# kubeflow/mpi-operator

Hardware: AMD Instinct MI355X
Metric: images/sec (higher is better)
Workload: dtype bf16; 1 GPU; model=resnet101, global_batch=64, image=224, parallelism=dp1, impl=hip, graph=True

## Files before the change

mpi_operator_amd/ops/_backend.py:

```python
from __future__ import annotations

import importlib
import os
import sys

_ext = None
_ext_err: Exception | None = None


def _try_load():
    global _ext, _ext_err
    if _ext is not None or _ext_err is not None:
        return
    try:
        import torch

        _ext = importlib.import_module("mpi_operator_amd.ops._mpi_amd_hip")
        if os.environ.get("MPIAMD_EPI_VEC", "1") == "0":
            _ext.set_epilogue_vec(False)
    except Exception as e:
        _ext_err = e


def hip_ext():
    _try_load()
    if _ext is None:
        raise RuntimeError(
            "mpi_operator_amd HIP extension (_mpi_amd_hip.so) is not available "
            "but a GPU op was requested. Build it in-tree with "
            "`python -m mpi_operator_amd.ops.build_hip` (hipcc, gfx950). "
            f"Original import error: {_ext_err!r}"
        )
    return _ext


def hip_available() -> bool:
    _try_load()
    return _ext is not None
```

mpi_operator_amd/ops/csrc/batchnorm.hip:

```cpp
#include "common.h"
#include "knobs.h"
#include "launchers.h"

template <int WHAT>
__global__ void bn_partials_k(const ushort8 *__restrict__ x,
                              const ushort8 *__restrict__ dy,
                              const ushort8 *__restrict__ y,
                              const uint8_t *__restrict__ mask,
                              const float *__restrict__ mean,
                              const float *__restrict__ invstd,
                              float *__restrict__ partial,
                              long M, int C8, int relu) {
  int C = C8 * 8;
  int cb = threadIdx.x % C8;
  int row_lane = threadIdx.x / C8;
  int rows_per_block = blockDim.x / C8;
  float a0[8] = {0}, a1[8] = {0};
  float mn[8], is[8];
  if (WHAT == 1 && row_lane < rows_per_block) {
#pragma unroll
    for (int j = 0; j < 8; ++j) {
      mn[j] = mean[cb * 8 + j];
      is[j] = invstd[cb * 8 + j];
    }
  }
  if (row_lane < rows_per_block) {
    long stride = (long)gridDim.x * rows_per_block;
    for (long row = (long)blockIdx.x * rows_per_block + row_lane; row < M;
         row += 2 * stride) {
      long r2 = row + stride;
      bool has2 = r2 < M;
      long off = row * C8 + cb, off2 = r2 * C8 + cb;
      float fx[8], fx2[8];
      ushort8 vx = x[off];
      ushort8 vx2 = has2 ? x[off2] : ushort8{0, 0, 0, 0, 0, 0, 0, 0};
      bf8_to_f8(vx, fx);
      bf8_to_f8(vx2, fx2);
      if (WHAT == 0) {
#pragma unroll
        for (int j = 0; j < 8; ++j) {
          a0[j] += fx[j] + fx2[j];
          a1[j] += fx[j] * fx[j] + fx2[j] * fx2[j];
        }
      } else {
        ushort8 vdy = dy[off];
        ushort8 vdy2 = has2 ? dy[off2] : ushort8{0, 0, 0, 0, 0, 0, 0, 0};
        float fdy[8], fdy2[8];
        bf8_to_f8(vdy, fdy);
        bf8_to_f8(vdy2, fdy2);
        if (relu) {
          if (mask) {
            int m1 = mask[off], m2 = has2 ? mask[off2] : 0;
#pragma unroll
            for (int j = 0; j < 8; ++j) {
              if (!(m1 & (1 << j))) fdy[j] = 0.f;
              if (!(m2 & (1 << j))) fdy2[j] = 0.f;
            }
          } else {
            ushort8 vy = y[off];
            ushort8 vy2 = has2 ? y[off2] : ushort8{0, 0, 0, 0, 0, 0, 0, 0};
#pragma unroll
            for (int j = 0; j < 8; ++j) {
              if (!(bf2f(vy[j]) > 0.f)) fdy[j] = 0.f;
              if (!(bf2f(vy2[j]) > 0.f)) fdy2[j] = 0.f;
            }
          }
        }
#pragma unroll
        for (int j = 0; j < 8; ++j) {
          a0[j] += fdy[j] + fdy2[j];
          a1[j] += fdy[j] * ((fx[j] - mn[j]) * is[j]) +
                   fdy2[j] * ((fx2[j] - mn[j]) * is[j]);
        }
      }
    }
  }
  __shared__ float lds[2][256 * 8];
#pragma unroll
  for (int j = 0; j < 8; ++j) {
    lds[0][threadIdx.x * 8 + j] = a0[j];
    lds[1][threadIdx.x * 8 + j] = a1[j];
  }
  __syncthreads();
  if (row_lane == 0) {
    for (int rl = 1; rl < rows_per_block; ++rl) {
// ... 395 lines not shown
      f2[j] = f2[j] * sc[j] + sh[j] + g2[j];
      if (relu) {
        if (f[j] > 0.f) m1 |= 1 << j;
        if (f2[j] > 0.f) m2 |= 1 << j;
        f[j] = fmaxf(f[j], 0.f);
        f2[j] = fmaxf(f2[j], 0.f);
      }
    }
    y[off] = f8_to_bf8(f);
    if (r2 < M) y[off2] = f8_to_bf8(f2);
    if (relu && mask) {
      mask[off] = (uint8_t)m1;
      if (r2 < M) mask[off2] = (uint8_t)m2;
    }
  }
}

__global__ void bn_bwd_apply_k(const ushort8 *__restrict__ dy,
                               const ushort8 *__restrict__ x,
                               const ushort8 *__restrict__ y,
                               const uint8_t *__restrict__ mask,
                               const float *__restrict__ mean,
                               const float *__restrict__ invstd,
                               const float *__restrict__ k1,
                               const float *__restrict__ k2,
                               const float *__restrict__ k3,
                               ushort8 *__restrict__ dx, long M, int C8,
                               int relu) {
  int cb = threadIdx.x % C8;
  int row_lane = threadIdx.x / C8;
  int rows_per_block = blockDim.x / C8;
  if (row_lane >= rows_per_block) return;
  float mn[8], is[8], a[8], b[8], c3[8];
#pragma unroll
  for (int j = 0; j < 8; ++j) {
    int c = cb * 8 + j;
    mn[j] = mean[c];
    is[j] = invstd[c];
    a[j] = k1[c];
    b[j] = k2[c];
    c3[j] = k3[c];
  }
  long stride = (long)gridDim.x * rows_per_block;
  for (long row = (long)blockIdx.x * rows_per_block + row_lane; row < M;
       row += 2 * stride) {
    long r2 = row + stride;
    long off = row * C8 + cb, off2 = r2 * C8 + cb;
    ushort8 vdy = dy[off], vx = x[off];
    ushort8 vdy2 = r2 < M ? dy[off2] : ushort8{0, 0, 0, 0, 0, 0, 0, 0};
    ushort8 vx2 = r2 < M ? x[off2] : ushort8{0, 0, 0, 0, 0, 0, 0, 0};
    float fdy[8], fx[8], fdy2[8], fx2[8];
    bf8_to_f8(vdy, fdy);
    bf8_to_f8(vx, fx);
    bf8_to_f8(vdy2, fdy2);
    bf8_to_f8(vx2, fx2);
    if (relu) {
      if (mask) {
        int m1 = mask[off], m2 = r2 < M ? mask[off2] : 0;
#pragma unroll
        for (int j = 0; j < 8; ++j) {
          if (!(m1 & (1 << j))) fdy[j] = 0.f;
          if (!(m2 & (1 << j))) fdy2[j] = 0.f;
        }
      } else {
        ushort8 vy = y[off];
        ushort8 vy2 = r2 < M ? y[off2] : ushort8{0, 0, 0, 0, 0, 0, 0, 0};
#pragma unroll
        for (int j = 0; j < 8; ++j) {
          if (!(bf2f(vy[j]) > 0.f)) fdy[j] = 0.f;
          if (!(bf2f(vy2[j]) > 0.f)) fdy2[j] = 0.f;
        }
      }
    }
#pragma unroll
    for (int j = 0; j < 8; ++j) {
      fdy[j] = a[j] * fdy[j] - b[j] - c3[j] * ((fx[j] - mn[j]) * is[j]);
      fdy2[j] = a[j] * fdy2[j] - b[j] - c3[j] * ((fx2[j] - mn[j]) * is[j]);
    }
    dx[off] = f8_to_bf8(fdy);
    if (r2 < M) dx[off2] = f8_to_bf8(fdy2);
  }
}

static void bn_geom(long M, int C8, int &grid, int &rows_per_block) {
  rows_per_block = 256 / C8;
  long g = (M + rows_per_block - 1) / rows_per_block;
  long cap = bn_grid_cap();
  grid = (int)(g > cap ? cap : (g < 1 ? 1 : g));
}

static int bn_apply_grid(long M, int C8) {
  const long cap = bn_apply_grid_cap();
  int rpb = 256 / C8;
  long g = (M + rpb - 1) / rpb;
  return (int)(g > cap ? cap : (g < 1 ? 1 : g));
}

extern "C" hipError_t bn_fwd_train_launch(
    const void *x, const void *res, const float *gamma, const float *beta,
    float eps, int relu, void *y, uint8_t *relu_mask, float *mean,
    float *invstd, float *scale, float *shift, float *partial,
    float *running_mean, float *running_var, float momentum, long M, int C,
    hipStream_t s) {
  int C8 = C / 8;
  if (C8 < 1 || C8 > 256) return hipErrorInvalidValue;
  int grid, rpb;
  bn_geom(M, C8, grid, rpb);
  bn_partials_k<0><<<grid, 256, 0, s>>>((const ushort8 *)x, nullptr, nullptr,
                                        nullptr, nullptr, nullptr, partial, M,
                                        C8, 0);
  HIP_KERNEL_CHECK();
  float unbias = M > 1 ? (float)M / (float)(M - 1) : 1.f;
  bn_finalize_fwd_bands_k<<<C, 256, 0, s>>>(
      partial, grid, C, gamma, beta, 1.f / (float)M, eps, mean, invstd, scale,
      shift, running_mean, running_var, momentum, unbias);
  HIP_KERNEL_CHECK();
  bn_apply_k<<<bn_apply_grid(M, C8), 256, 0, s>>>(
      (const ushort8 *)x, (const ushort8 *)res, scale, shift, (ushort8 *)y,
      relu_mask, M, C8, relu);
  HIP_KERNEL_CHECK();
  return hipSuccess;
}

__global__ void bn_finalize_fwd_bands_k(
    const float *__restrict__ partial, int grid, int C,
    const float *__restrict__ gamma, const float *__restrict__ beta,
    float inv_m, float eps, float *__restrict__ mean,
    float *__restrict__ invstd, float *__restrict__ scale,
    float *__restrict__ shift, float *__restrict__ running_mean,
    float *__restrict__ running_var, float momentum, float unbias) {
  int c = blockIdx.x;
  if (c >= C) return;
  float ga = 0.f, be = 0.f, rm = 0.f, rv = 0.f;
  if (threadIdx.x == 0) {
    ga = gamma[c];
    be = beta[c];
    if (running_mean) {
      rm = running_mean[c];
      rv = running_var[c];
    }
  }
  float s = 0.f, sq = 0.f;
  for (int g = threadIdx.x; g < grid; g += 256) {
    s += partial[(long)g * 2 * C + c];
    sq += partial[(long)g * 2 * C + C + c];
  }
  __shared__ float red[2][256 / WAVE];
  s = wave_sum(s);
  sq = wave_sum(sq);
  if ((threadIdx.x & (WAVE - 1)) == 0) {
    red[0][threadIdx.x / WAVE] = s;
    red[1][threadIdx.x / WAVE] = sq;
  }
  __syncthreads();
  if (threadIdx.x != 0) return;
  s = red[0][0] + red[0][1] + red[0][2] + red[0][3];
  sq = red[1][0] + red[1][1] + red[1][2] + red[1][3];
  float mu = s * inv_m;
  float var = fmaxf(sq * inv_m - mu * mu, 0.f);
  float is = rsqrtf(var + eps);
  mean[c] = mu;
  invstd[c] = is;
  float sc = ga * is;
  scale[c] = sc;
  shift[c] = be - mu * sc;
  if (running_mean) {
    running_mean[c] = rm * (1.f - momentum) + mu * momentum;
    running_var[c] = rv * (1.f - momentum) + var * unbias * momentum;
  }
}

extern "C" hipError_t bn_fwd_train_pre_launch(
    const float *pre_partial, int pre_grid, const void *x, const void *res,
    const float *gamma, const float *beta, float eps, int relu, void *y,
    uint8_t *relu_mask, float *mean, float *invstd, float *scale,
    float *shift, float *running_mean, float *running_var, float momentum,
    long M, int C, hipStream_t s) {
  int C8 = C / 8;
  if (C8 < 1 || C8 > 256) return hipErrorInvalidValue;
  float unbias = M > 1 ? (float)M / (float)(M - 1) : 1.f;
  bn_finalize_fwd_bands_k<<<C, 256, 0, s>>>(
      pre_partial, pre_grid, C, gamma, beta, 1.f / (float)M, eps, mean,
      invstd, scale, shift, running_mean, running_var, momentum, unbias);
  HIP_KERNEL_CHECK();
  bn_apply_k<<<bn_apply_grid(M, C8), 256, 0, s>>>(
      (const ushort8 *)x, (const ushort8 *)res, scale, shift, (ushort8 *)y,
      relu_mask, M, C8, relu);
  HIP_KERNEL_CHECK();
  return hipSuccess;
}

extern "C" hipError_t bn_fwd_eval_launch(const void *x, const float *scale,
                                         const float *shift, int relu, void *y,
                                         long M, int C, hipStream_t s) {
  int C8 = C / 8;
  if (C8 < 1 || C8 > 256) return hipErrorInvalidValue;
  int grid, rpb;
  bn_geom(M, C8, grid, rpb);
  bn_apply_k<<<bn_apply_grid(M, C8), 256, 0, s>>>(
      (const ushort8 *)x, nullptr, scale, shift, (ushort8 *)y, nullptr, M, C8,
      relu);
  HIP_KERNEL_CHECK();
  return hipSuccess;
}

extern "C" hipError_t bn_bwd_launch(const void *dy, const void *x,
                                    const void *y, const uint8_t *relu_mask,
                                    const float *gamma, const float *mean,
                                    const float *invstd, int relu, void *dx,
                                    float *dgamma, float *dbeta, float *k1,
                                    float *k2, float *k3, float *partial,
                                    long M, int C, hipStream_t s) {
  int C8 = C / 8;
  if (C8 < 1 || C8 > 256) return hipErrorInvalidValue;
  int grid, rpb;
  bn_geom(M, C8, grid, rpb);
  bn_partials_k<1><<<grid, 256, 0, s>>>((const ushort8 *)x, (const ushort8 *)dy,
                                        (const ushort8 *)y, relu_mask, mean,
                                        invstd, partial, M, C8, relu);
  HIP_KERNEL_CHECK();
  bn_finalize_bwd_bands_k<<<C, 256, 0, s>>>(
      partial, grid, C, gamma, invstd, 1.f / (float)M, dbeta, dgamma, k1, k2, k3);
  HIP_KERNEL_CHECK();
  bn_bwd_apply_k<<<bn_apply_grid(M, C8), 256, 0, s>>>(
      (const ushort8 *)dy, (const ushort8 *)x, (const ushort8 *)y, relu_mask,
      mean, invstd, k1, k2, k3, (ushort8 *)dx, M, C8, relu);
  HIP_KERNEL_CHECK();
  return hipSuccess;
}

extern "C" int bn_stats_grid(long M, int C) {
  int grid, rpb;
  bn_geom(M, C / 8, grid, rpb);
  return grid;
}

#define BN_RS_DISPATCH(WHAT, ...)                                              \
  do {                                                                         \
    switch (splits) {                                                          \
    case 2: bn_reduce_stats_k<WHAT, 2><<<grid, 256, 0, s>>>(__VA_ARGS__); break; \
    case 3: bn_reduce_stats_k<WHAT, 3><<<grid, 256, 0, s>>>(__VA_ARGS__); break; \
    case 4: bn_reduce_stats_k<WHAT, 4><<<grid, 256, 0, s>>>(__VA_ARGS__); break; \
    case 5: bn_reduce_stats_k<WHAT, 5><<<grid, 256, 0, s>>>(__VA_ARGS__); break; \
    case 6: bn_reduce_stats_k<WHAT, 6><<<grid, 256, 0, s>>>(__VA_ARGS__); break; \
    case 8: bn_reduce_stats_k<WHAT, 8><<<grid, 256, 0, s>>>(__VA_ARGS__); break; \
    case 16: bn_reduce_stats_k<WHAT, 16><<<grid, 256, 0, s>>>(__VA_ARGS__); break; \
    default: bn_reduce_stats_k<WHAT, 0><<<grid, 256, 0, s>>>(__VA_ARGS__); break; \
    }                                                                          \
  } while (0)

extern "C" hipError_t bn_reduce_stats_fwd_launch(const float *slabs,
                                                 int splits, void *y,
                                                 float *partial, long M, int C,
                                                 hipStream_t s) {
  int C8 = C / 8;
  if (C8 < 1 || C8 > 256 || C % 8 != 0 || splits < 2)
    return hipErrorInvalidValue;
  int grid, rpb;
  bn_geom(M, C8, grid, rpb);
  long len4 = M * C / 4;
  BN_RS_DISPATCH(0, (const float4v *)slabs, splits, len4, (ushort8 *)y,
                 nullptr, nullptr, nullptr, nullptr, nullptr, partial, M, C8,
                 0);
  return hipGetLastError();
}

extern "C" hipError_t bn_reduce_stats_bwd_launch(
    const float *slabs, int splits, void *dy, const void *x, const void *y,
    const uint8_t *relu_mask, const float *mean, const float *invstd, int relu,
    float *partial, long M, int C, hipStream_t s) {
  int C8 = C / 8;
  if (C8 < 1 || C8 > 256 || C % 8 != 0 || splits < 2)
    return hipErrorInvalidValue;
  int grid, rpb;
  bn_geom(M, C8, grid, rpb);
  long len4 = M * C / 4;
  BN_RS_DISPATCH(1, (const float4v *)slabs, splits, len4, (ushort8 *)dy,
                 (const ushort8 *)x, (const ushort8 *)y, relu_mask, mean,
                 invstd, partial, M, C8, relu);
  return hipGetLastError();
}
#undef BN_RS_DISPATCH

extern "C" hipError_t bn_join_stats_launch(
    const void *a, const uint8_t *jmask, const void *b, void *dxt,
    const uint8_t *cmask, const void *x, const float *mean,
    const float *invstd, float *partial, const void *xd, const float *mean_d,
    const float *invstd_d, float *partial_d, long M, int C, hipStream_t s) {
  int C8 = C / 8;
  if (C8 < 1 || C8 > 256 || C % 8 != 0 || M < 1 || !cmask)
    return hipErrorInvalidValue;
  if (xd && (!mean_d || !invstd_d || !partial_d)) return hipErrorInvalidValue;
  int grid, rpb;
  bn_geom(M, C8, grid, rpb);
#define BN_JS_LAUNCH(JOIN, NSTAT)                                              \
  bn_join_stats_k<JOIN, NSTAT><<<grid, 256, 0, s>>>(                           \
      (const ushort8 *)a, jmask, (const ushort8 *)b, (ushort8 *)dxt, cmask,    \
      (const ushort8 *)x, mean, invstd, partial, (const ushort8 *)xd, mean_d,  \
      invstd_d, partial_d, M, C8)
  if (jmask) {
    if (xd) BN_JS_LAUNCH(1, 2);
    else BN_JS_LAUNCH(1, 1);
  } else {
    if (xd) BN_JS_LAUNCH(0, 2);
    else BN_JS_LAUNCH(0, 1);
  }
#undef BN_JS_LAUNCH
  return hipGetLastError();
}

extern "C" hipError_t bn_bwd_pre_launch(
    const float *pre_partial, int pre_grid, const void *dy, const void *x,
    const void *y, const uint8_t *relu_mask, const float *gamma,
    const float *mean, const float *invstd, int relu, void *dx, float *dgamma,
    float *dbeta, float *k1, float *k2, float *k3, long M, int C,
    hipStream_t s) {
  int C8 = C / 8;
  if (C8 < 1 || C8 > 256) return hipErrorInvalidValue;
  bn_finalize_bwd_bands_k<<<C, 256, 0, s>>>(pre_partial, pre_grid, C, gamma,
                                            invstd, 1.f / (float)M, dbeta,
                                            dgamma, k1, k2, k3);
  HIP_KERNEL_CHECK();
  bn_bwd_apply_k<<<bn_apply_grid(M, C8), 256, 0, s>>>(
      (const ushort8 *)dy, (const ushort8 *)x, (const ushort8 *)y, relu_mask,
      mean, invstd, k1, k2, k3, (ushort8 *)dx, M, C8, relu);
  HIP_KERNEL_CHECK();
  return hipSuccess;
}
```

mpi_operator_amd/ops/csrc/bindings.cpp:

```cpp
#include <torch/extension.h>

#include <ATen/hip/impl/HIPGuardImplMasqueradingAsCUDA.h>
#include <ATen/hip/impl/HIPStreamMasqueradingAsCUDA.h>
#include <hip/hip_runtime.h>

#include <vector>

#include "knobs.h"
#include "launchers.h"

namespace {

using at::Tensor;

int conv_splits(long M, int Ncols, int K) {
  const int force = conv_splits_force();
  if (force >= 1) return force;
  long tiles = ((M + 127) / 128) * ((Ncols + 127) / 128);
  int nk = (K + 63) / 64;
  if (tiles >= 256 || nk < 16) return 1;
  long s = 512 / tiles;
  if (s > nk / 8) s = nk / 8;
  if (s > 16) s = 16;
  return s < 1 ? 1 : (int)s;
// ... 1235 lines not shown

static void lamb_step(std::vector<Tensor> masters, std::vector<Tensor> grads,
                      std::vector<Tensor> exp_avgs,
                      std::vector<Tensor> exp_avg_sqs, std::vector<Tensor> outs,
                      Tensor scalars, Tensor partials, Tensor ratio,
                      double beta1, double beta2, double eps, double wd,
                      bool adam_w_mode, double max_grad_norm) {
  TORCH_CHECK(!masters.empty());
  const HIPDeviceGuard guard(masters[0].device());
  OptGroups g = opt_groups(masters, grads, exp_avgs, exp_avg_sqs, outs, scalars);
  check_slab(partials, 3 * (int64_t)g.blocks, "partials");
  check_slab(ratio, g.tensors, "ratio");
  opt_tick(g, scalars, partials, beta1, beta2, max_grad_norm);
  float *pw = partials.data_ptr<float>() + g.blocks;
  float *pu = pw + g.blocks;
  int block_base = 0, tensor_base = 0;
  for (int t = 0; t < 2; ++t) {
    const auto &v = g.by_dtype[t];
    if (v.empty()) continue;
    CHK(lamb_step_launch(v.data(), (int)v.size(), t, scalars.data_ptr<float>(),
                         pw, pu, block_base, ratio.data_ptr<float>(),
                         tensor_base, beta1, beta2, eps, wd,
                         adam_w_mode ? 1 : 0, cur_stream()));
    block_base += optim_block_count(v.data(), (int)v.size());
    tensor_base += (int)v.size();
  }
}

static Tensor gemm_nt_b(const Tensor &a, const Tensor &b, bool c_f32) {
  const HIPDeviceGuard guard(a.device());
  Tensor ac = a.contiguous(), bc = b.contiguous();
  int M = ac.size(0), K = ac.size(1), N = bc.size(0);
  TORCH_CHECK(bc.size(1) == K);
  TORCH_CHECK(K % 8 == 0, "gemm_nt requires K%8==0");
  Tensor c = at::empty({M, N}, ac.options().dtype(c_f32 ? at::kFloat : at::kBFloat16));
  CHK(gemm_nt(ac.data_ptr(), bc.data_ptr(), c.data_ptr(), M, N, K, K, K, N,
              c_f32 ? 1 : 0, cur_stream()));
  return c;
}

static py::dict route_info() {
  py::dict d;
  d["pipemix"] = use_pipemix();
  d["pipe8"] = use_pipe8();
  d["p256x16"] = use_p256x16();
  d["gemm256"] = use_gemm256();
  d["pipe"] = use_pipe();
  d["pipent"] = use_pipent();
  d["glds"] = use_glds();
  d["onebuf"] = use_onebuf();
  d["splitmajor"] = use_splitmajor();
  d["sk_cpx"] = use_sk_cpx();
  d["fwd_sk"] = fwd_sk_on();
  d["dx_sk"] = dx_sk_mode();
  d["linear_sk"] = linear_sk_on();
  d["gelu_deriv"] = gelu_deriv_mode();
  d["gelubwd_wt"] = gelubwd_wt_on();
  d["pipegather"] = use_pipegather();
  d["pipegather_wgrad"] = use_pipegather_wgrad();
  d["pipes2"] = use_pipes2();
  d["ln_spec"] = ln_spec();
  d["ln2"] = ln2_mode();
  d["bn_grid"] = bn_grid_cap();
  d["bn_apply_grid"] = bn_apply_grid_cap();
  d["conv_splits_force"] = conv_splits_force();
  d["wgrad_budget"] = wgrad_budget();
  return d;
}

static const char *nt_route(int M, int N, int K, int splits) {
  static const char *const names[] = {"pipe256", "nt256", "pipemix", "glds",
                                      "reg"};
  int r = gemm_nt_route_id(M, N, K, splits);
  TORCH_CHECK(r >= 0 && r < 5, "unknown NT route id ", r);
  return names[r];
}

PYBIND11_MODULE(TORCH_EXTENSION_NAME, m) {
  m.def("route_info", &route_info);
  m.def("nt_route", &nt_route, py::arg("M"), py::arg("N"), py::arg("K"),
        py::arg("splits") = 1);
  m.def("set_epilogue_vec",
        [](bool on) { return gemm_set_epilogue_vec(on ? 1 : 0) != 0; });
  m.def("gelubwd_wt_route", [](int M, int N, int K) {
    return gemm_gelubwd_wants_wt(M, N, K) != 0;
  });
  m.def("conv_splits", [](int64_t M, int Ncols, int K) {
    return conv_splits((long)M, Ncols, K);
  }, py::arg("M"), py::arg("Ncols"), py::arg("K"));
  m.def("conv_wgrad_splits", [](int Kout, int RSC, int64_t M) {
    return wgrad_splits(Kout, RSC, (long)M);
  }, py::arg("Kout"), py::arg("RSC"), py::arg("M"));
  m.def("conv2d_fwd", &conv2d_fwd);
  m.def("conv2d_dgrad", &conv2d_dgrad);
  m.def("conv2d_fwd_bn", &conv2d_fwd_bn, py::arg("x"), py::arg("w"),
        py::arg("stride"), py::arg("pad"), py::arg("fuse_splitk") = true,
        py::arg("fuse_epilogue") = true);
  m.def("conv2d_dgrad_bn", &conv2d_dgrad_bn);
  m.def("bn_bwd_pre", &bn_bwd_pre);
  m.def("join_bwd_stats", &join_bwd_stats);
  m.def("bn_fwd_train_pre", &bn_fwd_train_pre);
  m.def("conv2d_wgrad", &conv2d_wgrad);
  m.def("conv2d_dgrad_acc", &conv2d_dgrad_acc);
  m.def("add_bf16", &add_bf16_b);
  m.def("bn_fwd_train", &bn_fwd_train);
  m.def("bn_fwd_eval", &bn_fwd_eval);
  m.def("bn_bwd", &bn_bwd);
  m.def("maxpool_fwd", &maxpool_fwd);
  m.def("maxpool_bwd", &maxpool_bwd);
  m.def("gap_fwd", &gap_fwd_b);
  m.def("gap_bwd", &gap_bwd_b);
  m.def("layernorm_fwd", &layernorm_fwd);
  m.def("layernorm_bwd", &layernorm_bwd);
  m.def("layernorm_add_fwd", &layernorm_add_fwd);
  m.def("linear_fwd", &linear_fwd);
  m.def("linear_bwd", &linear_bwd);
  m.def("linear_dgrad", &linear_dgrad);
  m.def("linear_dgrad_acc", &linear_dgrad_acc);
  m.def("softmax_xent_fwd", &softmax_xent_fwd);
  m.def("masked_xent_fwd", &masked_xent_fwd);
  m.def("mlm_head_fwd", &mlm_head_fwd);
  m.def("mlm_head_bwd", &mlm_head_bwd);
  m.def("linear_gelu_fwd", &linear_gelu_fwd);
  m.def("attn_fwd", &attn_fwd);
  m.def("attn_bwd", &attn_bwd);
  m.def("flash_attn_fwd", &flash_attn_fwd);
  m.def("flash_attn_bwd", &flash_attn_bwd);
  m.def("linear_wgrad_only", &linear_wgrad_only);
  m.def("linear_gelu_dgrad", &linear_gelu_dgrad);
  m.def("masked_xent_bwd", &masked_xent_bwd);
  m.def("softmax_xent_bwd", &softmax_xent_bwd);
  m.def("add_relu_fwd", &add_relu_fwd_b);
  m.def("add_relu_bwd", &add_relu_bwd_b);
  m.def("add_relu_bwd_add", &add_relu_bwd_add_b);
  m.def("add_relu_bwd_add_mask", &add_relu_bwd_add_mask_b);
  m.def("sgd_step", &sgd_step);
  m.def("adam_step", &adam_step);
  m.def("lamb_step", &lamb_step);
  m.def("gemm_nt", &gemm_nt_b);
  m.def("mfma_probe", [](const Tensor &a, const Tensor &b) {
    const HIPDeviceGuard guard(a.device());
    Tensor d = at::empty({16, 16}, a.options().dtype(at::kFloat));
    CHK(mfma_probe(a.contiguous().data_ptr(), b.contiguous().data_ptr(),
                   d.data_ptr<float>(), cur_stream()));
    return d;
  });
}
```

mpi_operator_amd/ops/csrc/launchers.h:

```cpp
#pragma once

#include <hip/hip_runtime.h>
#include <stdint.h>

struct SgdDesc {
  const void *grad;
  float *master;
  float *mom;
  uint16_t *out;
  long numel;
};

struct OptDesc {
  const void *grad;
  float *master;
  float *m;
  float *v;
  uint16_t *out;
  long numel;
};

extern "C" {

hipError_t add_bf16(const void *a, const void *b, void *c, long n,
                    hipStream_t s);
hipError_t add_relu_fwd(const void *a, const void *b, void *y, long n,
                        hipStream_t s);
hipError_t add_relu_bwd_add_mask(const void *dy, const void *mask,
                                 const void *dx0, void *dxt, long n,
                                 hipStream_t s);
hipError_t add_relu_bwd_add(const void *dy, const void *y, const void *dx0,
                            void *dxt, long n, hipStream_t s);
hipError_t add_relu_bwd(const void *dy, const void *y, void *dx, long n,
                        hipStream_t s);
hipError_t gap_fwd(const void *x, void *y, int N, int HW, int C,
                   hipStream_t s);
hipError_t gap_bwd(const void *dy, void *dx, int N, int HW, int C,
                   hipStream_t s);
hipError_t sgd_step_launch(const SgdDesc *descs, int nt, int grad_is_bf16,
                           float lr, float mu, float wd, int nesterov,
                           hipStream_t s);
hipError_t bias_add(void *y, const float *b, long M, int N, hipStream_t s);
int colsum_chunks(long M, int N);
hipError_t colsum_bf16(const void *dy, float *partial, float *db, long M,
                       int N, long ld, hipStream_t s);

hipError_t bn_fwd_train_launch(const void *x, const void *res,
                               const float *gamma, const float *beta,
                               float eps, int relu, void *y,
                               uint8_t *relu_mask, float *mean, float *invstd,
                               float *scale, float *shift, float *partial,
                               float *running_mean, float *running_var,
                               float momentum, long M, int C, hipStream_t s);
hipError_t bn_fwd_train_pre_launch(const float *pre_partial, int pre_grid,
                                   const void *x, const void *res,
                                   const float *gamma, const float *beta,
                                   float eps, int relu, void *y,
                                   uint8_t *relu_mask, float *mean,
                                   float *invstd, float *scale, float *shift,
                                   float *running_mean, float *running_var,
                                   float momentum, long M, int C,
                                   hipStream_t s);
hipError_t bn_fwd_eval_launch(const void *x, const float *scale,
                              const float *shift, int relu, void *y, long M,
                              int C, hipStream_t s);
hipError_t bn_bwd_launch(const void *dy, const void *x, const void *y,
                         const uint8_t *relu_mask, const float *gamma,
                         const float *mean, const float *invstd, int relu,
                         void *dx, float *dgamma, float *dbeta, float *k1,
                         float *k2, float *k3, float *partial, long M, int C,
                         hipStream_t s);
int bn_stats_grid(long M, int C);
hipError_t bn_reduce_stats_fwd_launch(const float *slabs, int splits, void *y,
                                      float *partial, long M, int C,
                                      hipStream_t s);
hipError_t bn_reduce_stats_bwd_launch(const float *slabs, int splits, void *dy,
                                      const void *x, const void *y,
                                      const uint8_t *relu_mask,
                                      const float *mean, const float *invstd,
                                      int relu, float *partial, long M, int C,
                                      hipStream_t s);
hipError_t bn_join_stats_launch(const void *a, const uint8_t *jmask,
                                const void *b, void *dxt, const uint8_t *cmask,
                                const void *x, const float *mean,
                                const float *invstd, float *partial,
                                const void *xd, const float *mean_d,
                                const float *invstd_d, float *partial_d,
                                long M, int C, hipStream_t s);
hipError_t bn_bwd_pre_launch(const float *pre_partial, int pre_grid,
                             const void *dy, const void *x, const void *y,
                             const uint8_t *relu_mask, const float *gamma,
                             const float *mean, const float *invstd, int relu,
                             void *dx, float *dgamma, float *dbeta, float *k1,
                             float *k2, float *k3, long M, int C,
                             hipStream_t s);

hipError_t maxpool_fwd_launch(const void *x, void *y, uint8_t *idx, int N,
                              int H, int W, int HO, int WO, int C, int K,
                              int stride, int pad, hipStream_t s);
hipError_t maxpool_bwd_launch(const void *dy, const uint8_t *idx, void *dx,
                              int N, int H, int W, int HO, int WO, int C,
                              int K, int stride, int pad, hipStream_t s);

hipError_t softmax_xent_fwd_launch(const void *logits, const long *target,
                                   float *probs, float *loss, int B, int V,
                                   hipStream_t s);
hipError_t softmax_xent_bwd_launch(const float *probs, const long *target,
                                   void *dlogits, int B, int V,
                                   const float *dscale, hipStream_t s);

hipError_t masked_xent_fwd_launch(const void *logits, const long *target,
                                  float *stats, float *out, int B, int V,
                                  long ld, long ignore_index, hipStream_t s);
hipError_t masked_xent_bwd_launch(const void *logits, const long *target,
                                  const float *stats, const float *out,
                                  const float *dscale, void *dlogits, int B,
                                  int V, long ld, long ignore_index,
                                  hipStream_t s);

hipError_t attn_fwd_launch(const void *qkv, void *ctx, void *probs,
                           const float *mask, int B, int S, int H, float scale,
                           hipStream_t strm);
hipError_t attn_bwd_launch(const void *qkv, const void *dctx,
                           const void *probs, void *dqkv, int B, int S, int H,
                           float scale, hipStream_t strm);

hipError_t flash_attn_fwd_launch(const void *qkv, void *ctx, float *lse,
                                 const float *mask, int B, int S, int H,
                                 float scale, hipStream_t strm);
hipError_t flash_attn_bwd_launch(const void *qkv, const void *ctx,
                                 const void *dctx, const float *lse,
                                 float *delta, const float *mask, void *dqkv,
                                 int B, int S, int H, float scale,
                                 hipStream_t strm);

hipError_t gemm_nt(const void *a, const void *b, void *c, int M, int N, int K,
                   long lda, long ldb, long ldc, int c_f32, hipStream_t s);
hipError_t gemm_nt_bias(const void *a, const void *b, const float *bias,
                        void *c, int M, int N, int K, long lda, long ldb,
                        long ldc, hipStream_t s);
int gemm_fwd_splits(int M, int N, int K);
hipError_t gemm_nt_bias_sk(const void *a, const void *b, const float *bias,
                           float *partial, void *c, int M, int N, int K,
                           long lda, long ldb, long ldc, int splits,
                           hipStream_t s);
hipError_t gemm_nt_gelu_bias(const void *x, const void *w, const float *bias,
                             void *deriv, void *g, int M, int N, int K,
                             long lda, long ldb, long ldc, hipStream_t s);
int gemm_gelubwd_wants_wt(int M, int N, int K);
hipError_t gemm_nt_tn_gelubwd(const void *dy, const void *w, const void *deriv,
                              void *dh, int M, int N, int K, long lda,
                              long ldb, long ldc, void *wt_buf, hipStream_t s);
hipError_t gemm_nt_tn_acc(const void *a, const void *b, void *c, int M, int N,
                          int K, long lda, long ldb, long ldc, hipStream_t s);
hipError_t gemm_nt_tn(const void *a, const void *b, void *c, int M, int N,
// ... 85 lines not shown
```

Before: 4084 images/sec.

## Add software-pipelined BN backward partials and coalesced multi-channel finalize kernels

```diff
diff --git a/mpi_operator_amd/ops/_backend.py b/mpi_operator_amd/ops/_backend.py
--- a/mpi_operator_amd/ops/_backend.py
+++ b/mpi_operator_amd/ops/_backend.py
@@ -18,6 +18,10 @@
         _ext = importlib.import_module("mpi_operator_amd.ops._mpi_amd_hip")
         if os.environ.get("MPIAMD_EPI_VEC", "1") == "0":
             _ext.set_epilogue_vec(False)
+        if os.environ.get("MPIAMD_BN_PIPELINED", "1") == "0":
+            _ext.set_bn_pipelined(False)
+        if os.environ.get("MPIAMD_BN_FINALIZE_COALESCED", "1") == "0":
+            _ext.set_bn_finalize_coalesced(False)
     except Exception as e:
         _ext_err = e
 
diff --git a/mpi_operator_amd/ops/csrc/batchnorm.hip b/mpi_operator_amd/ops/csrc/batchnorm.hip
--- a/mpi_operator_amd/ops/csrc/batchnorm.hip
+++ b/mpi_operator_amd/ops/csrc/batchnorm.hip
@@ -1,6 +1,7 @@
 #include "common.h"
 #include "knobs.h"
 #include "launchers.h"
+#include <atomic>
 
 template <int WHAT>
 __global__ void bn_partials_k(const ushort8 *__restrict__ x,
@@ -562,6 +563,421 @@
   }
 }
 
+#ifndef MPIAMD_BN_PIPE_DEPTH
+#define MPIAMD_BN_PIPE_DEPTH 1
+#endif
+constexpr int BN_PD = MPIAMD_BN_PIPE_DEPTH;
+constexpr unsigned BN_OOB = 0x80000000u;
+typedef __attribute__((ext_vector_type(4))) unsigned int uint4v;
+typedef __amdgpu_buffer_rsrc_t bn_rsrc_t;
+
+DEV_INLINE bn_rsrc_t bn_rsrc(const void *p, long bytes) {
+  return __builtin_amdgcn_make_buffer_rsrc((void *)p, 0, (int)bytes,
+                                           0x00020000);
+}
+DEV_INLINE ushort8 bn_ld16(bn_rsrc_t r, unsigned byte_off) {
+  return __builtin_bit_cast(
+      ushort8, __builtin_amdgcn_raw_buffer_load_b128(r, byte_off, 0, 0));
+}
+DEV_INLINE int bn_ld1(bn_rsrc_t r, unsigned byte_off) {
+  return (int)__builtin_amdgcn_raw_buffer_load_b8(r, byte_off, 0, 0);
+}
+DEV_INLINE void bn_st16(bn_rsrc_t r, unsigned byte_off, ushort8 v) {
+  __builtin_amdgcn_raw_buffer_store_b128(__builtin_bit_cast(uint4v, v), r,
+                                         byte_off, 0, 0);
+}
+DEV_INLINE unsigned bn_off(long row, long M, int C8, int cb) {
+  return row < M ? (unsigned)(row * C8 + cb) : BN_OOB;
+}
+DEV_INLINE unsigned bn_off16(unsigned e) {
+  return e == BN_OOB ? BN_OOB : e * 16;
+}
+
+DEV_INLINE void bn_acc_bwd_sel(float *a0, float *a1, const float *fx,
+                               const float *fx2, const float *fdy,
+                               const float *fdy2, const float *mn,
+                               const float *is, bool ok) {
+#pragma unroll
+  for (int j = 0; j < 8; ++j) {
+    float n0 = __fadd_rn(a0[j], __fadd_rn(fdy[j], fdy2[j]));
+    float xh = __fmul_rn(__fsub_rn(fx[j], mn[j]), is[j]);
+    float xh2 = __fmul_rn(__fsub_rn(fx2[j], mn[j]), is[j]);
+    float n1 =
+        __fadd_rn(a1[j], __fmaf_rn(fdy[j], xh, __fmul_rn(fdy2[j], xh2)));
+    a0[j] = ok ? n0 : a0[j];
+    a1[j] = ok ? n1 : a1[j];
+  }
+}
+
+DEV_INLINE void bn_gate(float *fdy, int m) {
+#pragma unroll
+  for (int j = 0; j < 8; ++j) fdy[j] = (m & (1 << j)) ? fdy[j] : 0.f;
+}
+
+struct BnPartialsStage {
+  ushort8 x, x2, dy, dy2;
+  int m, m2;
+};
+
+__global__ void __launch_bounds__(256)
+bn_partials_bwd_pipe_k(const ushort8 *__restrict__ x,
+                       const ushort8 *__restrict__ dy,
+                       const uint8_t *__restrict__ mask,
+                       const float *__restrict__ mean,
+                       const float *__restrict__ invstd,
+                       float *__restrict__ partial,
+                       long M, int C8) {
+  int cb = threadIdx.x % C8;
+  int row_lane = threadIdx.x / C8;
+  int rows_per_block = blockDim.x / C8;
+  float a0[8] = {0}, a1[8] = {0};
+  float mn[8], is[8];
+  if (row_lane < rows_per_block) {
+#pragma unroll
+    for (int j = 0; j < 8; ++j) {
+      mn[j] = mean[cb * 8 + j];
+      is[j] = invstd[cb * 8 + j];
+    }
+  }
+  if (row_lane < rows_per_block) {
+    const long stride = (long)gridDim.x * rows_per_block, step = 2 * stride;
+    const long nb = M * C8 * 16;
+    const bn_rsrc_t rx = bn_rsrc(x, nb), rdy = bn_rsrc(dy, nb);
+    const bn_rsrc_t rm = bn_rsrc(mask, M * C8);
+    auto load = [&](BnPartialsStage &b, long r) {
+      unsigned e = bn_off(r, M, C8, cb), e2 = bn_off(r + stride, M, C8, cb);
+      b.x = bn_ld16(rx, bn_off16(e));
+      b.x2 = bn_ld16(rx, bn_off16(e2));
+      b.dy = bn_ld16(rdy, bn_off16(e));
+      b.dy2 = bn_ld16(rdy, bn_off16(e2));
+      b.m = bn_ld1(rm, e);
+      b.m2 = bn_ld1(rm, e2);
+    };
+    BnPartialsStage buf[BN_PD + 1];
+    long row = (long)blockIdx.x * rows_per_block + row_lane;
+#pragma unroll
+    for (int k = 0; k < BN_PD; ++k) load(buf[k], row + k * step);
+    while (row < M) {
+#pragma unroll
+      for (int k = 0; k <= BN_PD; ++k) {
+        load(buf[(k + BN_PD) % (BN_PD + 1)], row + BN_PD * step);
+        __builtin_amdgcn_sched_barrier(0);
+        const BnPartialsStage &b = buf[k];
+        float fx[8], fx2[8], fdy[8], fdy2[8];
+        bf8_to_f8(b.x, fx);
+        bf8_to_f8(b.x2, fx2);
+        bf8_to_f8(b.dy, fdy);
+        bf8_to_f8(b.dy2, fdy2);
+        bn_gate(fdy, b.m);
+        bn_gate(fdy2, b.m2);
+        bn_acc_bwd_sel(a0, a1, fx, fx2, fdy, fdy2, mn, is, row < M);
+        row += step;
+        __builtin_amdgcn_sched_barrier(0);
+      }
+    }
+  }
+  bn_block_store(a0, a1, partial, C8, cb, row_lane, rows_per_block);
+}
+
+struct BnJoinStage {
+  ushort8 a, a2, b, b2, x, x2, xd, xd2;
+  int jm, jm2, cm, cm2;
+};
+
+template <int NSTAT>
+__global__ void __launch_bounds__(256)
+bn_join_stats_pipe_k(const ushort8 *__restrict__ a,
+                     const uint8_t *__restrict__ jmask,
+                     const ushort8 *__restrict__ b, ushort8 *__restrict__ dxt,
+                     const uint8_t *__restrict__ cmask,
+                     const ushort8 *__restrict__ x,
+                     const float *__restrict__ mean,
+                     const float *__restrict__ invstd,
+                     float *__restrict__ partial,
+                     const ushort8 *__restrict__ xd,
+                     const float *__restrict__ mean_d,
+                     const float *__restrict__ invstd_d,
+                     float *__restrict__ partial_d, long M, int C8) {
+  int cb = threadIdx.x % C8;
+  int row_lane = threadIdx.x / C8;
+  int rows_per_block = blockDim.x / C8;
+  float a0[8] = {0}, a1[8] = {0}, d0[8] = {0}, d1[8] = {0};
+  float mn[8], is[8], mnd[8], isd[8];
+  if (row_lane < rows_per_block) {
+#pragma unroll
+    for (int j = 0; j < 8; ++j) {
+      mn[j] = mean[cb * 8 + j];
+      is[j] = invstd[cb * 8 + j];
+      if (NSTAT == 2) {
+        mnd[j] = mean_d[cb * 8 + j];
+        isd[j] = invstd_d[cb * 8 + j];
+      }
+    }
+  }
+  if (row_lane < rows_per_block) {
+    const long stride = (long)gridDim.x * rows_per_block, step = 2 * stride;
+    const long nb = M * C8 * 16;
+    const bn_rsrc_t ra = bn_rsrc(a, nb), rb = bn_rsrc(b, nb);
+    const bn_rsrc_t rx = bn_rsrc(x, nb), ro = bn_rsrc(dxt, nb);
+    const bn_rsrc_t rxd = bn_rsrc(xd, NSTAT == 2 ? nb : 0);
+    const bn_rsrc_t rjm = bn_rsrc(jmask, M * C8), rcm = bn_rsrc(cmask, M * C8);
+    auto load = [&](BnJoinStage &s, long r) {
+      unsigned e = bn_off(r, M, C8, cb), e2 = bn_off(r + stride, M, C8, cb);
+      unsigned o = bn_off16(e), o2 = bn_off16(e2);
+      s.a = bn_ld16(ra, o);
+      s.b = bn_ld16(rb, o);
+      s.x = bn_ld16(rx, o);
+      s.a2 = bn_ld16(ra, o2);
+      s.b2 = bn_ld16(rb, o2);
+      s.x2 = bn_ld16(rx, o2);
+      if (NSTAT == 2) {
+        s.xd = bn_ld16(rxd, o);
+        s.xd2 = bn_ld16(rxd, o2);
+      }
+      s.jm = bn_ld1(rjm, e);
+      s.jm2 = bn_ld1(rjm, e2);
+      s.cm = bn_ld1(rcm, e);
+      s.cm2 = bn_ld1(rcm, e2);
+    };
+    BnJoinStage buf[BN_PD + 1];
+    long row = (long)blockIdx.x * rows_per_block + row_lane;
+#pragma unroll
+    for (int k = 0; k < BN_PD; ++k) load(buf[k], row + k * step);
+    while (row < M) {
+#pragma unroll
+      for (int k = 0; k <= BN_PD; ++k) {
+        load(buf[(k + BN_PD) % (BN_PD + 1)], row + BN_PD * step);
+        __builtin_amdgcn_sched_barrier(0);
+        const BnJoinStage &s = buf[k];
+        ushort8 vo, vo2;
+#pragma unroll
+        for (int j = 0; j < 8; ++j) {
+          float g = (s.jm & (1 << j)) ? bf2f(s.a[j]) : 0.f;
+          float g2 = (s.jm2 & (1 << j)) ? bf2f(s.a2[j]) : 0.f;
+          vo[j] = f2bf(g + bf2f(s.b[j]));
+          vo2[j] = f2bf(g2 + bf2f(s.b2[j]));
+        }
+        bn_st16(ro, bn_off16(bn_off(row, M, C8, cb)), vo);
+        bn_st16(ro, bn_off16(bn_off(row + stride, M, C8, cb)), vo2);
+        float fo[8], fo2[8], fx[8], fx2[8];
+        bf8_to_f8(vo, fo);
+        bf8_to_f8(vo2, fo2);
+        bf8_to_f8(s.x, fx);
+        bf8_to_f8(s.x2, fx2);
+        bn_gate(fo, s.cm);
+        bn_gate(fo2, s.cm2);
+        bn_acc_bwd_sel(a0, a1, fx, fx2, fo, fo2, mn, is, row < M);
+        if (NSTAT == 2) {
+          float fxd[8], fxd2[8];
+          bf8_to_f8(s.xd, fxd);
+          bf8_to_f8(s.xd2, fxd2);
+          bn_acc_bwd_sel(d0, d1, fxd, fxd2, fo, fo2, mnd, isd, row < M);
+        }
+        row += step;
+        __builtin_amdgcn_sched_barrier(0);
+      }
+    }
+  }
+  bn_block_store(a0, a1, partial, C8, cb, row_lane, rows_per_block);
+  if (NSTAT == 2) {
+    __syncthreads();
+    bn_block_store(d0, d1, partial_d, C8, cb, row_lane, rows_per_block);
+  }
+}
+
+template <int CH>
+DEV_INLINE bool bn_fin_co_sums(const float *__restrict__ partial, int grid,
+                               int C, float &r0, float &r1) {
+  constexpr int RG = 256 / CH, KK = CH / 4;
+  const int ch = threadIdx.x % CH, rg = threadIdx.x / CH;
+  const int c = blockIdx.x * CH + ch;
+  const bn_rsrc_t rp = bn_rsrc(partial, (long)grid * 2 * C * 4);
+  float p0[CH], p1[CH];
+#pragma unroll
+  for (int k = 0; k < CH; ++k) p0[k] = p1[k] = 0.f;
+  for (int base = 0; base < grid; base += 256) {
+    float v0[CH], v1[CH];
+#pragma unroll
+    for (int k = 0; k < CH; ++k) {
+      int g = base + rg + k * RG;
+      bool ok = g < grid && c < C;
+      unsigned o = ok ? ((unsigned)g * 2 * C + c) * 4 : BN_OOB;
+      unsigned o1 = ok ? ((unsigned)g * 2 * C + C + c) * 4 : BN_OOB;
+      v0[k] = __builtin_bit_cast(
+          float, __builtin_amdgcn_raw_buffer_load_b32(rp, o, 0, 0));
+      v1[k] = __builtin_bit_cast(
+          float, __builtin_amdgcn_raw_buffer_load_b32(rp, o1, 0, 0));
+    }
+#pragma unroll
+    for (int k = 0; k < CH; ++k) {
+      bool ok = base + rg + k * RG < grid;
+      p0[k] = ok ? p0[k] + v0[k] : p0[k];
+      p1[k] = ok ? p1[k] + v1[k] : p1[k];
+    }
+  }
+  __shared__ float red[2 * 4 * 256];
+  __shared__ float red2[2 * 4 * CH];
+#pragma unroll
+  for (int w = 0; w < 4; ++w) {
+#pragma unroll
+    for (int off = KK / 2; off > 0; off >>= 1) {
+#pragma unroll
+      for (int kk = 0; kk < off; ++kk) {
+        p0[w * KK + kk] += p0[w * KK + kk + off];
+        p1[w * KK + kk] += p1[w * KK + kk + off];
+      }
+    }
+    red[((0 * 4 + w) * RG + rg) * CH + ch] = p0[w * KK];
+    red[((1 * 4 + w) * RG + rg) * CH + ch] = p1[w * KK];
+  }
+  __syncthreads();
+  if (threadIdx.x < 8 * CH) {
+    const int q = threadIdx.x / CH;
+    float v[RG];
+#pragma unroll
+    for (int r = 0; r < RG; ++r) v[r] = red[(q * RG + r) * CH + ch];
+#pragma unroll
+    for (int off = RG / 2; off > 0; off >>= 1) {
+#pragma unroll
+      for (int r = 0; r < off; ++r) v[r] += v[r + off];
+    }
+    red2[q * CH + ch] = v[0];
+  }
+  __syncthreads();
+  if (threadIdx.x >= CH || c >= C) return false;
+  r0 = red2[0 * CH + ch] + red2[1 * CH + ch] + red2[2 * CH + ch] +
+       red2[3 * CH + ch];
+  r1 = red2[4 * CH + ch] + red2[5 * CH + ch] + red2[6 * CH + ch] +
+       red2[7 * CH + ch];
+  return true;
+}
+
+template <int CH>
+__global__ void __launch_bounds__(256) bn_finalize_fwd_co_k(
+    const float *__restrict__ partial, int grid, int C,
+    const float *__restrict__ gamma, const float *__restrict__ beta,
+    float inv_m, float eps, float *__restrict__ mean,
+    float *__restrict__ invstd, float *__restrict__ scale,
+    float *__restrict__ shift, float *__restrict__ running_mean,
+    float *__restrict__ running_var, float momentum, float unbias) {
+  const int c = blockIdx.x * CH + threadIdx.x;
+  float ga = 0.f, be = 0.f, rm = 0.f, rv = 0.f;
+  if (threadIdx.x < CH && c < C) {
+    ga = gamma[c];
+    be = beta[c];
+    if (running_mean) {
+      rm = running_mean[c];
+      rv = running_var[c];
+    }
+  }
+  float s, sq;
+  if (!bn_fin_co_sums<CH>(partial, grid, C, s, sq)) return;
+  float mu = __fmul_rn(s, inv_m);
+  float var = fmaxf(__fmaf_rn(-mu, mu, __fmul_rn(sq, inv_m)), 0.f);
+  float is = rsqrtf(__fadd_rn(var, eps));
+  mean[c] = mu;
+  invstd[c] = is;
+  float sc = __fmul_rn(ga, is);
+  scale[c] = sc;
+  shift[c] = __fmaf_rn(-mu, sc, be);
+  if (running_mean) {
+    float keep = __fsub_rn(1.f, momentum);
+    running_mean[c] =
+        __fadd_rn(__fmul_rn(rm, keep), __fmul_rn(mu, momentum));
+    running_var[c] = __fadd_rn(
+        __fmul_rn(rv, keep), __fmul_rn(__fmul_rn(var, unbias), momentum));
+  }
+}
+
+template <int CH>
+__global__ void __launch_bounds__(256) bn_finalize_bwd_co_k(
+    const float *__restrict__ partial, int grid, int C,
+    const float *__restrict__ gamma, const float *__restrict__ invstd,
+    float inv_m, float *__restrict__ dbeta, float *__restrict__ dgamma,
+    float *__restrict__ k1, float *__restrict__ k2, float *__restrict__ k3) {
+  const int c = blockIdx.x * CH + threadIdx.x;
+  float ga = 0.f, iv = 0.f;
+  if (threadIdx.x < CH && c < C) {
+    ga = gamma[c];
+    iv = invstd[c];
+  }
+  float s0, s1;
+  if (!bn_fin_co_sums<CH>(partial, grid, C, s0, s1)) return;
+  dbeta[c] = s0;
+  dgamma[c] = s1;
+  float g_is = __fmul_rn(ga, iv);
+  k1[c] = g_is;
+  k2[c] = __fmul_rn(__fmul_rn(g_is, s0), inv_m);
+  k3[c] = __fmul_rn(__fmul_rn(g_is, s1), inv_m);
+}
+
+static std::atomic<bool> g_bn_pipelined{true};
+static std::atomic<bool> g_bn_finalize_co{true};
+static std::atomic<int> g_bn_finalize_ch{0};
+
+extern "C" int bn_set_pipelined(int on) {
+  return g_bn_pipelined.exchange(on != 0) ? 1 : 0;
+}
+extern "C" int bn_set_finalize_coalesced(int on) {
+  return g_bn_finalize_co.exchange(on != 0) ? 1 : 0;
+}
+extern "C" int bn_set_finalize_ch(int ch) {
+  if (ch != 0 && ch != -1 && ch != 8 && ch != 16) return -2;
+  return g_bn_finalize_ch.exchange(ch);
+}
+
+static bool bn_pipe_ok(long M, int C8, int grid, int rows_per_block) {
+  return g_bn_pipelined.load(std::memory_order_relaxed) &&
+         M * C8 * 16 < (1L << 31) && M > 4L * grid * rows_per_block;
+}
+
+static int bn_fin_ch(int C, int grid) {
+  if (!g_bn_finalize_co.load(std::memory_order_relaxed)) return 0;
+  if ((long)grid * 2 * C * 4 >= (1L << 31)) return 0;
+  int forced = g_bn_finalize_ch.load(std::memory_order_relaxed);
+  if (forced) return forced < 0 ? 0 : forced;
+  if (C < 256) return 0;
+  return C >= 2048 || (C >= 512 && grid > 1024) ? 16 : 8;
+}
+
+static void bn_finalize_fwd_dispatch(
+    const float *partial, int grid, int C, const float *gamma,
+    const float *beta, float inv_m, float eps, float *mean, float *invstd,
+    float *scale, float *shift, float *running_mean, float *running_var,
+    float momentum, float unbias, hipStream_t s) {
+#define BN_FIN_FWD(CH)                                                         \
+  bn_finalize_fwd_co_k<CH><<<(C + CH - 1) / CH, 256, 0, s>>>(                  \
+      partial, grid, C, gamma, beta, inv_m, eps, mean, invstd, scale, shift,   \
+      running_mean, running_var, momentum, unbias)
+  switch (bn_fin_ch(C, grid)) {
+  case 8: BN_FIN_FWD(8); break;
+  case 16: BN_FIN_FWD(16); break;
+  default:
+    bn_finalize_fwd_bands_k<<<C, 256, 0, s>>>(
+        partial, grid, C, gamma, beta, inv_m, eps, mean, invstd, scale, shift,
+        running_mean, running_var, momentum, unbias);
+  }
+#undef BN_FIN_FWD
+}
+
+static void bn_finalize_bwd_dispatch(const float *partial, int grid, int C,
+                                     const float *gamma, const float *invstd,
+                                     float inv_m, float *dbeta, float *dgamma,
+                                     float *k1, float *k2, float *k3,
+                                     hipStream_t s) {
+#define BN_FIN_BWD(CH)                                                         \
+  bn_finalize_bwd_co_k<CH><<<(C + CH - 1) / CH, 256, 0, s>>>(                  \
+      partial, grid, C, gamma, invstd, inv_m, dbeta, dgamma, k1, k2, k3)
+  switch (bn_fin_ch(C, grid)) {
+  case 8: BN_FIN_BWD(8); break;
+  case 16: BN_FIN_BWD(16); break;
+  default:
+    bn_finalize_bwd_bands_k<<<C, 256, 0, s>>>(partial, grid, C, gamma, invstd,
+                                              inv_m, dbeta, dgamma, k1, k2, k3);
+  }
+#undef BN_FIN_BWD
+}
+
 static void bn_geom(long M, int C8, int &grid, int &rows_per_block) {
   rows_per_block = 256 / C8;
   long g = (M + rows_per_block - 1) / rows_per_block;
@@ -591,9 +1007,9 @@
                                         C8, 0);
   HIP_KERNEL_CHECK();
   float unbias = M > 1 ? (float)M / (float)(M - 1) : 1.f;
-  bn_finalize_fwd_bands_k<<<C, 256, 0, s>>>(
-      partial, grid, C, gamma, beta, 1.f / (float)M, eps, mean, invstd, scale,
-      shift, running_mean, running_var, momentum, unbias);
+  bn_finalize_fwd_dispatch(partial, grid, C, gamma, beta, 1.f / (float)M, eps,
+                           mean, invstd, scale, shift, running_mean,
+                           running_var, momentum, unbias, s);
   HIP_KERNEL_CHECK();
   bn_apply_k<<<bn_apply_grid(M, C8), 256, 0, s>>>(
       (const ushort8 *)x, (const ushort8 *)res, scale, shift, (ushort8 *)y,
@@ -659,9 +1075,9 @@
   int C8 = C / 8;
   if (C8 < 1 || C8 > 256) return hipErrorInvalidValue;
   float unbias = M > 1 ? (float)M / (float)(M - 1) : 1.f;
-  bn_finalize_fwd_bands_k<<<C, 256, 0, s>>>(
-      pre_partial, pre_grid, C, gamma, beta, 1.f / (float)M, eps, mean,
-      invstd, scale, shift, running_mean, running_var, momentum, unbias);
+  bn_finalize_fwd_dispatch(pre_partial, pre_grid, C, gamma, beta,
+                           1.f / (float)M, eps, mean, invstd, scale, shift,
+                           running_mean, running_var, momentum, unbias, s);
   HIP_KERNEL_CHECK();
   bn_apply_k<<<bn_apply_grid(M, C8), 256, 0, s>>>(
       (const ushort8 *)x, (const ushort8 *)res, scale, shift, (ushort8 *)y,
@@ -695,12 +1111,17 @@
   if (C8 < 1 || C8 > 256) return hipErrorInvalidValue;
   int grid, rpb;
   bn_geom(M, C8, grid, rpb);
-  bn_partials_k<1><<<grid, 256, 0, s>>>((const ushort8 *)x, (const ushort8 *)dy,
-                                        (const ushort8 *)y, relu_mask, mean,
-                                        invstd, partial, M, C8, relu);
+  if (relu && relu_mask && bn_pipe_ok(M, C8, grid, rpb))
+    bn_partials_bwd_pipe_k<<<grid, 256, 0, s>>>(
+        (const ushort8 *)x, (const ushort8 *)dy, relu_mask, mean, invstd,
+        partial, M, C8);
+  else
+    bn_partials_k<1><<<grid, 256, 0, s>>>((const ushort8 *)x, (const ushort8 *)dy,
+                                          (const ushort8 *)y, relu_mask, mean,
+                                          invstd, partial, M, C8, relu);
   HIP_KERNEL_CHECK();
-  bn_finalize_bwd_bands_k<<<C, 256, 0, s>>>(
-      partial, grid, C, gamma, invstd, 1.f / (float)M, dbeta, dgamma, k1, k2, k3);
+  bn_finalize_bwd_dispatch(partial, grid, C, gamma, invstd, 1.f / (float)M,
+                           dbeta, dgamma, k1, k2, k3, s);
   HIP_KERNEL_CHECK();
   bn_bwd_apply_k<<<bn_apply_grid(M, C8), 256, 0, s>>>(
       (const ushort8 *)dy, (const ushort8 *)x, (const ushort8 *)y, relu_mask,
@@ -773,11 +1194,18 @@
   if (xd && (!mean_d || !invstd_d || !partial_d)) return hipErrorInvalidValue;
   int grid, rpb;
   bn_geom(M, C8, grid, rpb);
+  const bool pipe = jmask && bn_pipe_ok(M, C8, grid, rpb);
+#define BN_JS_ARGS                                                             \
+  (const ushort8 *)a, jmask, (const ushort8 *)b, (ushort8 *)dxt, cmask,        \
+      (const ushort8 *)x, mean, invstd, partial, (const ushort8 *)xd, mean_d,  \
+      invstd_d, partial_d, M, C8
 #define BN_JS_LAUNCH(JOIN, NSTAT)                                              \
-  bn_join_stats_k<JOIN, NSTAT><<<grid, 256, 0, s>>>(                           \
-      (const ushort8 *)a, jmask, (const ushort8 *)b, (ushort8 *)dxt, cmask,    \
-      (const ushort8 *)x, mean, invstd, partial, (const ushort8 *)xd, mean_d,  \
-      invstd_d, partial_d, M, C8)
+  do {                                                                         \
+    if (pipe)                                                                  \
+      bn_join_stats_pipe_k<NSTAT><<<grid, 256, 0, s>>>(BN_JS_ARGS);            \
+    else                                                                       \
+      bn_join_stats_k<JOIN, NSTAT><<<grid, 256, 0, s>>>(BN_JS_ARGS);           \
+  } while (0)
   if (jmask) {
     if (xd) BN_JS_LAUNCH(1, 2);
     else BN_JS_LAUNCH(1, 1);
@@ -786,6 +1214,7 @@
     else BN_JS_LAUNCH(0, 1);
   }
 #undef BN_JS_LAUNCH
+#undef BN_JS_ARGS
   return hipGetLastError();
 }
 
@@ -797,9 +1226,8 @@
     hipStream_t s) {
   int C8 = C / 8;
   if (C8 < 1 || C8 > 256) return hipErrorInvalidValue;
-  bn_finalize_bwd_bands_k<<<C, 256, 0, s>>>(pre_partial, pre_grid, C, gamma,
-                                            invstd, 1.f / (float)M, dbeta,
-                                            dgamma, k1, k2, k3);
+  bn_finalize_bwd_dispatch(pre_partial, pre_grid, C, gamma, invstd,
+                           1.f / (float)M, dbeta, dgamma, k1, k2, k3, s);
   HIP_KERNEL_CHECK();
   bn_bwd_apply_k<<<bn_apply_grid(M, C8), 256, 0, s>>>(
       (const ushort8 *)dy, (const ushort8 *)x, (const ushort8 *)y, relu_mask,
diff --git a/mpi_operator_amd/ops/csrc/bindings.cpp b/mpi_operator_amd/ops/csrc/bindings.cpp
--- a/mpi_operator_amd/ops/csrc/bindings.cpp
+++ b/mpi_operator_amd/ops/csrc/bindings.cpp
@@ -1341,6 +1341,15 @@
         py::arg("splits") = 1);
   m.def("set_epilogue_vec",
         [](bool on) { return gemm_set_epilogue_vec(on ? 1 : 0) != 0; });
+  m.def("set_bn_pipelined",
+        [](bool on) { return bn_set_pipelined(on ? 1 : 0) != 0; });
+  m.def("set_bn_finalize_coalesced",
+        [](bool on) { return bn_set_finalize_coalesced(on ? 1 : 0) != 0; });
+  m.def("set_bn_finalize_ch", [](int ch) {
+    int prev = bn_set_finalize_ch(ch);
+    TORCH_CHECK(prev != -2, "set_bn_finalize_ch: ch must be 0, -1, 8 or 16");
+    return prev;
+  });
   m.def("gelubwd_wt_route", [](int M, int N, int K) {
     return gemm_gelubwd_wants_wt(M, N, K) != 0;
   });
diff --git a/mpi_operator_amd/ops/csrc/launchers.h b/mpi_operator_amd/ops/csrc/launchers.h
--- a/mpi_operator_amd/ops/csrc/launchers.h
+++ b/mpi_operator_amd/ops/csrc/launchers.h
@@ -71,6 +71,9 @@
                          float *k2, float *k3, float *partial, long M, int C,
                          hipStream_t s);
 int bn_stats_grid(long M, int C);
+int bn_set_pipelined(int on);
+int bn_set_finalize_coalesced(int on);
+int bn_set_finalize_ch(int ch);
 hipError_t bn_reduce_stats_fwd_launch(const float *slabs, int splits, void *y,
                                       float *partial, long M, int C,
                                       hipStream_t s);
```

Result: faster. 4197 images/sec (median of 6 runs) (+2.8%).
